# WanqingXia/UR-gym

Measured on AMD Instinct MI355X. Metric: env-steps/sec (whole node), higher is better.
Workload: dtype f64; 1 GPU; UR5DynReach-v1 N=65536 per GPU, random actions U(-1,1), auto-reset, seed 0; envs_total=65536, gather_obs=False, rollout_api=False, gjk_start=bullet

## Files before the change

### ur_gym_amd/csrc/urgym_hip.hip

```cpp
#include <hip/hip_runtime.h>
#include <stdint.h>
#include <stdio.h>
#include <string.h>
#include <math.h>
#include <new>
#include <vector>

#include "../../include/urgym.h"
#include "../../data/ur5e_model.h"
#include "urgym_device.h"
#include "urgym_launch_plan.h"
#include "urgym_actor.h"
#include "urgym_critic.h"
#include "urgym_tables_host.h"

using namespace urgym;


namespace {

constexpr int WAVES = 4;
constexpr int THREADS = GROUP * WAVES;
constexpr uint32_t NO_ITEM = 0xFFFFFFFFu;
constexpr int REFILL_MIN = 16;
constexpr int RESIDENT = 3;
constexpr int SC_ROWS = 19;
constexpr int PAIR_TABLE = 0, PAIR_TRACK = 5, PAIR_SELF = 10;
__host__ __device__ constexpr int self_pair_bit(int la, int lb) {
  return PAIR_SELF + (la == 1 ? 0 : (la == 2 ? 4 : 7)) + (lb - (la + 2));
}

enum { MODE_STEP = 0, MODE_RESET = 1, MODE_REFRESH = 2, MODE_PREFETCH = 3 };
enum { Q_TABLE = 0, Q_TRACK = 1, Q_SELF = 2 };

constexpr double M_HULL = 0.001, M_PRIM = 0.001;
constexpr double CYL_R = 0.05, CYL_H = 0.4, M_CYL = M_PRIM;
constexpr double TABLE_CX = 0.5, TABLE_CY = 0.0, TABLE_CZ = -0.58, TABLE_HX = 0.55, TABLE_HY = 0.9, TABLE_HZ = 0.46;
constexpr double M_TABLE = M_PRIM;
constexpr double TRACK_CX = 0.0, TRACK_CY = 0.0, TRACK_CZ = -0.06, TRACK_HX = 0.1, TRACK_HY = 0.55, TRACK_HZ = 0.06;
constexpr double M_TRACK = M_PRIM;
constexpr double TARGET_BOX_H = 0.025, M_TARGET_BOX = M_PRIM, TARGET_SPHERE_R = 0.02;

struct DevTables {
  double joint_rot[6][9];
  double joint_xyz[6][3];
  double capsule[6][7];
};
__constant__ DevTables c_tab;

constexpr int REC_FIELDS = 36;
enum { REC_GOAL = 0, REC_START = 6, REC_END = 12, REC_VEL = 18, REC_QUAT = 24, REC_LD = 28, REC_DP = 33 };

struct KParams {
  urgym_config cfg;
  urgym_buffers buf;
  HullMap graph;
  int obs_dim, goal_dim;
  uint32_t seed_lo, seed_hi;
  int pp;
  int copy_final;
  int envs;
  int big_blocks;
  int envs_tail;
  double* rec_d;
  int32_t* rec_i;
  int2* rlist;
  int* rcount;
  int rcap;
  double* ld_scratch;
  double* sc_scratch;
  int* rzero;
  int* rzero2;
  int fallback_on;
  int prefetch;
  int inline_ori;
  float neutral_ach[6];
};
__device__ __forceinline__ double& REC(const KParams& P, int slot, int f, int n) {
  return P.rec_d[((size_t)slot * REC_FIELDS + f) * P.cfg.num_envs + n];
}
__device__ __forceinline__ int32_t& RECI(const KParams& P, int slot, int j, int n) {
  return P.rec_i[((size_t)slot * 2 + j) * P.cfg.num_envs + n];
}

__device__ __forceinline__ double& SOA(double* base, int f, int n, int N) { return base[(size_t)f * N + n]; }

__device__ __forceinline__ long long sortable(double x) {
  const long long k = __double_as_longlong(x);
  return k ^ ((k >> 63) & 0x7FFFFFFFFFFFFFFFLL);
}
__device__ __forceinline__ double unsortable(long long k) { return __longlong_as_double(k ^ ((k >> 63) & 0x7FFFFFFFFFFFFFFFLL)); }

__device__ __forceinline__ ShapeDesc hull_desc(int link ) {
  ShapeDesc s;
  s.type = SH_HULL; s.hull = link - 1; s.hx = s.hy = s.hz = 0.0;
  return s;
}
__device__ __forceinline__ ShapeDesc cyl_desc() {
  ShapeDesc s;
  s.type = SH_CYLZ; s.hull = 0;
  s.hx = s.hy = CYL_R - M_CYL; s.hz = 0.5 * CYL_H - M_CYL;
  return s;
}
__device__ __forceinline__ ShapeDesc box_desc(double hx, double hy, double hz, double margin) {
  ShapeDesc s;
  s.type = SH_BOX; s.hull = 0;
  s.hx = hx - margin; s.hy = hy - margin; s.hz = hz - margin;
  return s;
}
// ... 282 lines not shown
    integrate_obstacle(opos, oq, ovel, dp, cfg.dt);
  }
  if (KIND == URGYM_ENV_STA) {
    double st[6], en[6];
    bool moving = false;
    for (int i = 0; i < 6; i++) { st[i] = SOA(B.obst_start, i, n, N); en[i] = SOA(B.obst_end, i, n, N); moving = moving || en[i] != 0.0; }
    if (moving) {
      const double dx = en[0] - opos[0], dy = en[1] - opos[1], dz = en[2] - opos[2];
      double ovel[6] = {0, 0, 0, 0, 0, 0}, dp[3];
      if (sqrt(dx * dx + dy * dy + dz * dz) > 0.05) dyn_velocity(st, en, 1.0, ovel);
      step_displacement(ovel, cfg.dt, dp);
      integrate_obstacle(opos, oq, ovel, dp, cfg.dt);
    }
  }
}

template <int MODE>
struct EnvLds {
  static constexpr int ME = (MODE == MODE_PREFETCH) ? PREFETCH_MAX_ENVS : ((MODE == MODE_STEP) ? STEP_MAX_ENVS : MAX_ENVS);
  static constexpr bool LDS_Q = (MODE == MODE_REFRESH);
  static constexpr bool DIST_LDS = (MODE != MODE_STEP);
  static constexpr bool LDS_STATE = (MODE != MODE_STEP);
  double s_dist[5][DIST_LDS ? ME : 1];
  double s_q[LDS_Q ? 6 : 1][LDS_Q ? ME : 1];
  double s_obst[LDS_STATE ? 7 : 1][LDS_STATE ? ME : 1];
  uint32_t s_pairs[ME];
  int s_flags[ME];
  int s_env[ME];
  alignas(16) int s_ticket;
  int s_pending;
  int s_p1done;
  int s_left;
  int s_key[(MODE != MODE_STEP) ? ME : 1];
  double s_kind[(MODE == MODE_STEP) ? 8 : 1][5];
  double s_pose[GJK_SLOT_DOUBLES][THREADS];
};

template <int KIND, int MODE, bool WITH_EPA>
__device__ __forceinline__ void env_body(const KParams& P, const float* __restrict__ actions, EnvLds<MODE>& L, const int bidx, const int nblk) {
  constexpr int ME = EnvLds<MODE>::ME;
  constexpr bool LDS_Q = EnvLds<MODE>::LDS_Q, DIST_LDS = EnvLds<MODE>::DIST_LDS, LDS_STATE = EnvLds<MODE>::LDS_STATE;
  auto& s_dist = L.s_dist;
  auto& s_q = L.s_q;
  auto& s_obst = L.s_obst;
  auto& s_pairs = L.s_pairs;
  auto& s_flags = L.s_flags;
  auto& s_env = L.s_env;
  int& s_ticket = L.s_ticket;
  int& s_pending = L.s_pending;
  int& s_p1done = L.s_p1done;
  int& s_left = L.s_left;
  auto& s_key = L.s_key;
  auto& s_pose = L.s_pose;

  const urgym_config& cfg = P.cfg;
  const urgym_buffers& B = P.buf;
  const int N = cfg.num_envs;
  const int tid = threadIdx.x;
  const int lane = tid & 63;
  const int wv = __builtin_amdgcn_readfirstlane(tid >> 6);
  constexpr int OD = (KIND == URGYM_ENV_ORI) ? 18 : ((KIND == URGYM_ENV_OBS) ? 26 : ((KIND == URGYM_ENV_STA) ? 29 : 35));
  constexpr int GD = (KIND == URGYM_ENV_OBS) ? 3 : 6;
  int vb = bidx;
  if (MODE == MODE_STEP && P.envs_tail == 0) {
    const int nb = nblk, x = vb & 7, per = nb >> 3, rem = nb & 7;
    vb = x * per + (x < rem ? x : rem) + (vb >> 3);
  }
  const bool tail_block = (MODE == MODE_STEP) && P.envs_tail > 0 && vb >= P.big_blocks;
  const int E = tail_block ? P.envs_tail : P.envs;
  const int first = tail_block ? P.big_blocks * P.envs + (vb - P.big_blocks) * P.envs_tail : vb * P.envs;
  const int G = (E + GROUP - 1) / GROUP;
  constexpr bool HAS_OBST = (KIND != URGYM_ENV_ORI);
  constexpr int COLL_BIT = 1 << 30;
  constexpr int EE_BIT = 1 << 29;
  constexpr int EPA_SHIFT = 8, EPA_MASK = 0x7FFF << EPA_SHIFT;
  const bool need_epa = WITH_EPA && ((KIND == URGYM_ENV_OBS) || !cfg.check_collision || (MODE != MODE_STEP));
  XRef pose_slot{(URGYM_LDS double*)&s_pose[0][0] + tid, THREADS};
  float* const s_out = reinterpret_cast<float*>(&s_pose[0][0]);
  static_assert(sizeof(float) * STEP_MAX_ENVS * 47 <= sizeof(double) * GJK_SLOT_DOUBLES * THREADS, "staging must fit");
  auto dist_cell = [&](int i, int e) -> double* {
    return DIST_LDS ? (double*)&s_dist[i][DIST_LDS ? e : 0] : &P.ld_scratch[(size_t)i * N + first + e];
  };

  if (bidx == 0 && tid == 0) {
    if (P.rzero) *P.rzero = 0;
    if (P.rzero2) *P.rzero2 = 0;
  }
  int list_count = 0;
  if (MODE != MODE_STEP) {
    list_count = (MODE == MODE_PREFETCH) ? min(*P.rcount, P.rcap) : B.done_count[P.pp];
    if (first >= list_count) return;
  }
  if (tid == 0) { s_ticket = THREADS; s_pending = 0; s_p1done = 0; s_left = 0; }
  if (MODE == MODE_STEP && tid < 8) {
    const int k = tid & 3, ex = tid >> 2;
    const bool tbl = (k == Q_TABLE);
    const double msum = M_HULL + ((k == 3) ? M_CYL : ((k == Q_SELF) ? M_HULL : (tbl ? M_TABLE : M_TRACK)));
    const bool wants = (k == 3) || ex;
    const double verdict = wants ? 0.0 : msum + cfg.collision_margin;
    L.s_kind[tid][0] = (k == 3) ? (CYL_R - M_CYL) : (tbl ? (TABLE_HX - M_TABLE) : (TRACK_HX - M_TRACK));
    L.s_kind[tid][1] = (k == 3) ? (CYL_R - M_CYL) : (tbl ? (TABLE_HY - M_TABLE) : (TRACK_HY - M_TRACK));
    L.s_kind[tid][2] = (k == 3) ? (0.5 * CYL_H - M_CYL) : (tbl ? (TABLE_HZ - M_TABLE) : (TRACK_HZ - M_TRACK));
    L.s_kind[tid][3] = wants ? msum + 0.02 + 5.0 : verdict;
    L.s_kind[tid][4] = verdict;
  }
  const bool workbench = (KIND != URGYM_ENV_ORI) && cfg.link_dist_scope == URGYM_LINK_DIST_WORKBENCH;
  if (workbench && tid < E && (DIST_LDS || first + tid < N))
    for (int i = 0; i < 5; i++) *dist_cell(i, tid) = __longlong_as_double(0x7FF0000000000000LL);
  if (MODE == MODE_STEP && tid < E) {
    s_env[tid] = (first + tid < N) ? first + tid : -1;
    s_flags[tid] = 0;
    s_pairs[tid] = 0;
  }
  __syncthreads();
  const int p1_slot = (MODE == MODE_STEP) ? (wv - (WAVES - G)) * GROUP + lane : lane;
  const bool p1_lane = ((MODE == MODE_STEP) ? (wv >= WAVES - G) : (wv == 0)) && (p1_slot < E);
  int n_slot = -1, flags_slot = 0;
  int key_slot = 0;
  if (p1_lane) {
    const int idx = first + p1_slot;
    if (MODE == MODE_STEP) n_slot = idx < N ? idx : -1;
    else if (MODE == MODE_PREFETCH) {
      if (idx < list_count) { const int2 ent = P.rlist[idx]; n_slot = ent.x; key_slot = ent.y; }
    } else n_slot = idx < list_count ? B.done_list[idx] : -1;
  }
  if ((MODE == MODE_RESET || MODE == MODE_PREFETCH) && wv == 0) {
    int episode_used = 0;
    sample_episode_wave<KIND>(P, pose_slot, E, lane, n_slot, key_slot, MODE == MODE_PREFETCH, flags_slot, episode_used);
    if (p1_lane) s_key[p1_slot] = (MODE == MODE_PREFETCH) ? key_slot : episode_used + 1;
  }
  if (p1_lane) {
    const int e = p1_slot;
    const int n = n_slot;
    int flags = flags_slot;
    double q[6] = {0, 0, 0, 0, 0, 0};
    double opos[3] = {0, 0, 0};
    Q4 oq{0, 0, 0, 1};
    bool finite = true;
    if (n >= 0) {
      for (int i = 0; i < 6; i++) q[i] = joint_of_step<MODE>(P, actions, n, i);
      for (int i = 0; i < 6; i++) finite = finite && (fabs(q[i]) < 1.0e6);
      if (MODE == MODE_STEP) {
        bool over = false;
        for (int i = 0; i < 6; i++) over = over || (fabs(q[i]) > (i == 2 ? 3.141592653589793 : 6.283185307179586));
        if (over) atomicOr(&s_flags[p1_slot], URGYM_STATUS_JOINT_LIMIT);
      }
      if (HAS_OBST && LDS_STATE) {
        double sp[6];
        for (int i = 0; i < 6; i++) sp[i] = (MODE == MODE_PREFETCH) ? REC(P, key_slot & 1, REC_START + i, n) : SOA(B.obst_start, i, n, N);
        for (int i = 0; i < 3; i++) opos[i] = sp[i];
        oq = quat_from_rpy(sp[3], sp[4], sp[5]);
      }
    }
    const bool live = (n >= 0 && finite);
    const bool use_cache = (MODE == MODE_STEP) && (HAS_OBST || cfg.check_collision);
    if (use_cache && live) {
#pragma unroll 1
      for (int k = 0; k < 6; k++) {
        double sn, cs;
        sincos(joint_of_step<MODE>(P, actions, n, k), &sn, &cs);
        SOA(P.sc_scratch, 2 * k, n, N) = sn;
        SOA(P.sc_scratch, 2 * k + 1, n, N) = cs;
      }
      if (HAS_OBST) {
        obstacle_of_step<KIND>(P, n, opos, oq);
        for (int i = 0; i < 3; i++) SOA(P.sc_scratch, 12 + i, n, N) = opos[i];
        SOA(P.sc_scratch, 15, n, N) = oq.x; SOA(P.sc_scratch, 16, n, N) = oq.y; SOA(P.sc_scratch, 17, n, N) = oq.z; SOA(P.sc_scratch, 18, n, N) = oq.w;
      }
    }
    s_env[e] = live ? n : (n >= 0 ? -2 - n : -1);
    if (MODE != MODE_STEP) s_flags[e] = flags;
    if (LDS_STATE) {
      if (LDS_Q) for (int i = 0; i < 6; i++) s_q[i][e] = q[i];
      s_obst[0][e] = opos[0]; s_obst[1][e] = opos[1]; s_obst[2][e] = opos[2];
      s_obst[3][e] = oq.x; s_obst[4][e] = oq.y; s_obst[5][e] = oq.z; s_obst[6][e] = oq.w;
    }
    if (HAS_OBST && !live && (DIST_LDS || n >= 0))
      for (int i = 0; i < 5; i++) *dist_cell(i, e) = (n >= 0) ? __builtin_nan("") : 1e30;
    uint32_t pairs = 0;
    if (live && cfg.check_collision && MODE != MODE_RESET && MODE != MODE_PREFETCH) {
      const double lim = cfg.collision_margin + M_HULL + 1e-6;
      X3 T = identity_x3();
      D3 a0[3], a1[3];
#pragma unroll
      for (int k = 0; k < 6; k++) {
        double sn, cs;
        if (use_cache) { sn = SOA(P.sc_scratch, 2 * k, n, N); cs = SOA(P.sc_scratch, 2 * k + 1, n, N); }
        else sincos(q[k], &sn, &cs);
        fk_joint(T, k, sn, cs);
        const int link = k + 1;
        const double* c = c_tab.capsule[k];
        const D3 b0 = apply(T, d3(c[0], c[1], c[2])), b1 = apply(T, d3(c[3], c[4], c[5]));
        const double rb = c[6];
        if (k < 3) { a0[k] = b0; a1[k] = b1; }
        if (link >= 2) {
          if (seg_box_lower_bound(b0, b1, TABLE_CX, TABLE_CY, TABLE_CZ, TABLE_HX, TABLE_HY, TABLE_HZ) - rb <= lim) pairs |= 1u << (PAIR_TABLE + link - 2);
          if (seg_box_lower_bound(b0, b1, TRACK_CX, TRACK_CY, TRACK_CZ, TRACK_HX, TRACK_HY, TRACK_HZ) - rb <= lim) pairs |= 1u << (PAIR_TRACK + link - 2);
        }
#pragma unroll
        for (int A = 1; A <= 3; A++) {
          if (A <= link - 2) {
            if (segseg_dist(a0[A - 1], a1[A - 1], b0, b1) - c_tab.capsule[A - 1][6] - rb <= lim + M_HULL) pairs |= 1u << self_pair_bit(A, link);
          }
        }
      }
      if (MODE == MODE_STEP) {
        double er, ep, ey;
        rpy_from_quat(rot_to_quat(T.r), er, ep, ey);
        float* orow = B.observation + (size_t)n * OD;
        orow[0] = (float)T.t.x; orow[1] = (float)T.t.y; orow[2] = (float)T.t.z;
        orow[3] = (float)er; orow[4] = (float)ep; orow[5] = (float)ey;
        atomicOr(&s_flags[e], EE_BIT);
      }
    }
    s_pairs[e] = pairs;
    if (pairs) atomicAdd(&s_pending, __popc(pairs));
  }
  if (MODE == MODE_STEP) {
    if (wv >= WAVES - G && lane == 0) __hip_atomic_fetch_add(&s_p1done, 1, __ATOMIC_RELEASE, __HIP_MEMORY_SCOPE_WORKGROUP);
  } else {
    __syncthreads();
  }

  if (!(MODE == MODE_STEP && !HAS_OBST && !cfg.check_collision)) {
    D3 v0 = d3(0, 1, 0);
    int kind = 3, e = 0, lb = 2, la = 1;
    auto shape_a = [&]() -> ShapeDesc { return hull_desc(kind == Q_SELF ? la : lb); };
    auto shape_b = [&]() -> ShapeDesc {
      ShapeDesc s;
      s.type = (kind == 3) ? SH_CYLZ : ((kind == Q_SELF) ? SH_HULL : SH_BOX);
      s.hull = lb - 1;
      const bool tbl = (kind == Q_TABLE);
      s.hx = (kind == 3) ? (CYL_R - M_CYL) : (tbl ? (TABLE_HX - M_TABLE) : (TRACK_HX - M_TRACK));
      s.hy = (kind == 3) ? (CYL_R - M_CYL) : (tbl ? (TABLE_HY - M_TABLE) : (TRACK_HY - M_TRACK));
      s.hz = (kind == 3) ? (0.5 * CYL_H - M_CYL) : (tbl ? (TABLE_HZ - M_TABLE) : (TRACK_HZ - M_TRACK));
      return s;
    };
    bool exact = false;
    const bool guided = cfg.gjk_start == URGYM_GJK_START_GUIDED;
    auto capsule_mid = [&](int link, const X3& TX) -> D3 {
      const double* c = c_tab.capsule[link - 1];
      return apply(TX, d3(0.5 * (c[0] + c[3]), 0.5 * (c[1] + c[4]), 0.5 * (c[2] + c[5])));
    };
    auto guided_axis = [&](D3 mid, D3 centre) -> D3 {
      const D3 d = mid - centre;
      const double n2 = dot(d, d);
      return n2 > 1e-12 ? d * (1.0 / sqrt(n2)) : d3(0, 1, 0);
    };
    bool p1_ok = false;
    auto setup = [&](uint32_t item) -> bool {
      e = item & 255;
      kind = (item >> 8) & 3;
      exact = ((item >> 16) & 1) != 0;
      lb = (item >> 10) & 7;
      la = (item >> 13) & 7;
      if (e >= E || lb < 1 || lb > 6 || (kind == Q_SELF && (la < 1 || la > 6))) return false;
      const int n = s_env[e];
      if (n < 0) return false;
      const bool cached = (MODE == MODE_STEP) && p1_ok;
      if (MODE == MODE_STEP && !cached) {
        bool finite = true;
        for (int k = 0; k < 6; k++) finite = finite && (fabs(joint_of_step<MODE>(P, actions, n, k)) < 1.0e6);
        if (!finite) return false;
      }
      X3 T = identity_x3(), TA = identity_x3();
#pragma unroll 1
      for (int k = 0; k < lb; k++) {
        double sn, cs;
        if (cached) { sn = SOA(P.sc_scratch, 2 * k, n, N); cs = SOA(P.sc_scratch, 2 * k + 1, n, N); }
        else sincos(LDS_Q ? s_q[k][e] : joint_of_step<MODE>(P, actions, n, k), &sn, &cs);
        fk_joint(T, k, sn, cs);
        if (k + 1 == la) TA = T;
      }
      if (kind == 3) {
        X3 To;
        if (LDS_STATE) {
          quat_to_rot(Q4{s_obst[3][e], s_obst[4][e], s_obst[5][e], s_obst[6][e]}, To.r);
          To.t = d3(s_obst[0][e], s_obst[1][e], s_obst[2][e]);
        } else if (cached) {
          quat_to_rot(Q4{SOA(P.sc_scratch, 15, n, N), SOA(P.sc_scratch, 16, n, N), SOA(P.sc_scratch, 17, n, N), SOA(P.sc_scratch, 18, n, N)}, To.r);
          To.t = d3(SOA(P.sc_scratch, 12, n, N), SOA(P.sc_scratch, 13, n, N), SOA(P.sc_scratch, 14, n, N));
        } else {
          double op[3];
          Q4 oqs;
          obstacle_of_step<KIND>(P, n, op, oqs);
          quat_to_rot(oqs, To.r);
          To.t = d3(op[0], op[1], op[2]);
        }
        store(pose_slot, rel(To, T));
        v0 = rotT(To, guided ? guided_axis(capsule_mid(lb, T), To.t) : d3(0, 1, 0));
      } else if (kind == Q_SELF) {
        store(pose_slot, rel(T, TA));
        v0 = rotT(T, guided ? guided_axis(capsule_mid(la, TA), capsule_mid(lb, T)) : d3(0, 1, 0));
      } else {
        const bool tbl = (kind == Q_TABLE);
        const D3 centre = d3(tbl ? TABLE_CX : TRACK_CX, tbl ? TABLE_CY : TRACK_CY, tbl ? TABLE_CZ : TRACK_CZ);
        v0 = guided ? guided_axis(capsule_mid(lb, T), centre) : d3(0, 1, 0);
        T.t = T.t - centre;
        store(pose_slot, T);
      }
      return true;
    };
    auto claim_pair = [&]() -> uint32_t {
      int pe = tid % E;
#pragma unroll 1
      for (int trip = 0; trip < 2 * ME; trip++, pe = (pe + 1 == E ? 0 : pe + 1)) {
        uint32_t m = s_pairs[pe];
        while (m) {
          const int b = __ffs((int)m) - 1;
          const uint32_t old = atomicAnd(&s_pairs[pe], ~(1u << b));
          if (old & (1u << b)) {
            if (b < PAIR_TRACK) return (uint32_t)pe | (Q_TABLE << 8) | ((uint32_t)(b - PAIR_TABLE + 2) << 10);
            if (b < PAIR_SELF) return (uint32_t)pe | (Q_TRACK << 8) | ((uint32_t)(b - PAIR_TRACK + 2) << 10);
            const int i = b - PAIR_SELF;
            const int la = i < 4 ? 1 : (i < 7 ? 2 : 3);
            const int l2 = i < 4 ? 3 + i : (i < 7 ? i : i - 2);
            return (uint32_t)pe | (Q_SELF << 8) | ((uint32_t)l2 << 10) | ((uint32_t)la << 13);
          }
          m = old & ~(1u << b);
        }
      }
      return NO_ITEM;
    };
    auto margin_sum = [&]() -> double {
      return M_HULL + ((kind == 3) ? M_CYL : ((kind == Q_SELF) ? M_HULL : ((kind == Q_TABLE) ? M_TABLE : M_TRACK)));
    };
    const int n_tickets = HAS_OBST ? (workbench ? 15 : 5) * E : 0;
    auto ticket_item = [&](int t) -> uint32_t {
      const int body = t / (5 * E), r = t - body * 5 * E;
      const int tl = r / E, te = r - tl * E, link = 2 + tl;
      if (body == 0) return (uint32_t)te | (3u << 8) | ((uint32_t)link << 10);
      return (uint32_t)te | ((uint32_t)(body == 1 ? Q_TABLE : Q_TRACK) << 8) | ((uint32_t)link << 10) | (1u << 16);
    };

    GjkRun run;
    bool busy = false;
    if (MODE == MODE_STEP) p1_ok = __hip_atomic_load(&s_p1done, __ATOMIC_ACQUIRE, __HIP_MEMORY_SCOPE_WORKGROUP) >= G;
    if (tid < n_tickets) {
      busy = setup(ticket_item(tid));
      if (busy) gjk_begin(run, v0);
    }
    for (;;) {
      if (busy) {
        if (MODE == MODE_STEP) {
          const URGYM_LDS double* row = (const URGYM_LDS double*)(URGYM_LDS void*)&L.s_kind[kind | ((int)exact << 2)][0];
          ShapeDesc sb;
          sb.type = (kind == 3) ? SH_CYLZ : ((kind == Q_SELF) ? SH_HULL : SH_BOX);
          sb.hull = lb - 1;
          sb.hx = row[0]; sb.hy = row[1]; sb.hz = row[2];
          gjk_iterate(run, P.graph, shape_a(), pose_slot, sb, row[3], row[4]);
        } else {
          const bool wants_distance = (kind == 3 || exact);
          const double verdict_d = wants_distance ? 0.0 : margin_sum() + cfg.collision_margin;
          gjk_iterate(run, P.graph, shape_a(), pose_slot, shape_b(), wants_distance ? margin_sum() + 0.02 + 5.0 : verdict_d, verdict_d);
        }
        if (run.done) {
          const double msum = margin_sum();
          if (kind == 3 || exact) {
            double dist = run.core - msum;
            if (run.info & GJK_PENETRATING) {
              dist = -msum;
              const int body = (kind == 3) ? 0 : (kind == Q_TABLE ? 1 : 2);
              atomicOr(&s_flags[e], URGYM_STATUS_PENETRATION | (need_epa ? (1 << (EPA_SHIFT + 5 * body + (lb - 2))) : 0));
            }
            if (run.info & GJK_ITERCAP) atomicOr(&s_flags[e], URGYM_STATUS_GJK_ITER);
            if (workbench) atomicMin(reinterpret_cast<long long*>(dist_cell(lb - 2, e)), sortable(dist));
            else *dist_cell(lb - 2, e) = dist;
          } else {
            const bool hit = (run.info & (GJK_PENETRATING | GJK_CLOSE)) || (!(run.info & GJK_SEPARATED) && (run.core - msum) <= cfg.collision_margin);
            if (hit) atomicOr(&s_flags[e], COLL_BIT);
          }
          busy = false;
        }
      }
      typedef int pool_words __attribute__((ext_vector_type(4)));
      const pool_words pool = *(volatile URGYM_LDS pool_words*)(URGYM_LDS void*)&s_ticket;
      __builtin_amdgcn_fence(__ATOMIC_ACQUIRE, "workgroup");
      const bool more_tickets = pool.x < n_tickets;
      const bool p1_published = (MODE != MODE_STEP) || pool.z >= G;
      const bool more_pairs = pool.y > 0;
      if (MODE == MODE_STEP) p1_ok = p1_published;
      const int idle_lanes = __popcll(__ballot(!busy));
      if (!busy && (idle_lanes >= REFILL_MIN || idle_lanes == 64)) {
        uint32_t item = NO_ITEM;
        if (more_tickets) {
          const int t = atomicAdd(&s_ticket, 1);
          if (t < n_tickets) item = ticket_item(t);
        } else if (more_pairs) {
          if (atomicSub(&s_pending, 1) > 0) item = claim_pair();
        }
        if (item != NO_ITEM) {
          busy = setup(item);
          if (busy) gjk_begin(run, v0);
        }
      }
      if (__ballot(busy) == 0ull && !more_tickets && !more_pairs && p1_published) break;
    }
    auto epa_pass = [&]() -> bool {
      const EpaWs ws{(URGYM_LDS double*)&s_pose[0][0] + GROUP * wv, THREADS};
      bool armed = false;
#pragma unroll 1
      for (int g = 0; g < G; g++) {
        const int sl = g * GROUP + lane;
        const int marks = (sl < E) ? ((__hip_atomic_load(&s_flags[sl], __ATOMIC_RELAXED, __HIP_MEMORY_SCOPE_WORKGROUP) & EPA_MASK) >> EPA_SHIFT) : 0;
        unsigned long long envs_marked = __ballot(marks != 0);
#pragma unroll 1
        while (envs_marked) {
          const int el = __builtin_ctzll(envs_marked);
          envs_marked &= envs_marked - 1ull;
          const int ee = g * GROUP + el;
          int me = __shfl(marks, el);
#pragma unroll 1
          while (me) {
            const int b = __builtin_ctz((unsigned)me);
            me &= me - 1;
            int mine = 0;
            if (lane == 0) mine = (atomicAnd(&s_flags[ee], ~(1 << (EPA_SHIFT + b))) >> (EPA_SHIFT + b)) & 1;
            if (!__shfl(mine, 0)) continue;
            if (!armed) {
              pose_slot.p = ws.base;
              if (MODE == MODE_STEP) p1_ok = true;
              armed = true;
            }
            const int body = b / 5, link = 2 + b - 5 * body;
            const uint32_t item = (uint32_t)ee | ((uint32_t)(body == 0 ? 3 : (body == 1 ? Q_TABLE : Q_TRACK)) << 8) | ((uint32_t)link << 10) |
                                  ((body ? 1u : 0u) << 16);
            if (!setup(item)) continue;
            epa_wave_sync();
            bool capped;
            const double depth = epa_wave(P.graph, shape_a(), shape_b(), ws, lane, capped);
            if (lane == 0) {
              const double dist = -(depth + margin_sum());
              if (workbench) atomicMin(reinterpret_cast<long long*>(dist_cell(lb - 2, e)), sortable(dist));
              else *dist_cell(lb - 2, e) = dist;
              if (capped) atomicOr(&s_flags[e], URGYM_STATUS_GJK_ITER);
            }
          }
        }
      }
      if (armed) pose_slot.p = (URGYM_LDS double*)&s_pose[0][0] + tid;
      return armed;
    };
    if (HAS_OBST && WITH_EPA) {
      if (lane == 0) __hip_atomic_fetch_add(&s_left, 1, __ATOMIC_RELEASE, __HIP_MEMORY_SCOPE_WORKGROUP);
#pragma unroll 1
      for (;;) {
        const int left = __hip_atomic_load(&s_left, __ATOMIC_ACQUIRE, __HIP_MEMORY_SCOPE_WORKGROUP);
        const bool served = epa_pass();
        if (!served && left >= WAVES) break;
        if (!served) __builtin_amdgcn_s_sleep(16);
      }
    }
    __syncthreads();
  }

  const int pe = (wv - (WAVES - G)) * GROUP + lane;
  if (wv >= WAVES - G && pe < E && s_env[pe] != -1) {
    const int n = s_env[pe] >= 0 ? s_env[pe] : -2 - s_env[pe];
    double q[6];
    for (int i = 0; i < 6; i++) q[i] = LDS_Q ? s_q[i][pe] : joint_of_step<MODE>(P, actions, n, i);
    const bool ee_ready = (MODE == MODE_STEP) && (s_flags[pe] & EE_BIT);
    X3 TE = identity_x3();
    if (!ee_ready) {
      if (KIND == URGYM_ENV_ORI) {
        double sn[6], cs[6];
#pragma unroll
        for (int k = 0; k < 6; k++) sincos(q[k], &sn[k], &cs[k]);
#pragma unroll
        for (int k = 0; k < 6; k++) fk_joint(TE, k, sn[k], cs[k]);
      } else {
#pragma unroll 1
        for (int k = 0; k < 6; k++) {
          double sn, cs;
          sincos(q[k], &sn, &cs);
          fk_joint(TE, k, sn, cs);
        }
      }
    }
    double opos[3] = {0, 0, 0};
    Q4 oq{0, 0, 0, 1};
    if (HAS_OBST) {
      if (LDS_STATE) {
        opos[0] = s_obst[0][pe]; opos[1] = s_obst[1][pe]; opos[2] = s_obst[2][pe];
        oq = Q4{s_obst[3][pe], s_obst[4][pe], s_obst[5][pe], s_obst[6][pe]};
      } else if (s_env[pe] >= 0) {
        for (int i = 0; i < 3; i++) opos[i] = SOA(P.sc_scratch, 12 + i, n, N);
        oq = Q4{SOA(P.sc_scratch, 15, n, N), SOA(P.sc_scratch, 16, n, N), SOA(P.sc_scratch, 17, n, N), SOA(P.sc_scratch, 18, n, N)};
      } else {
        obstacle_of_step<KIND>(P, n, opos, oq);
      }
    }
    const int step_count = B.step_count[n];
    float* row = &s_out[pe * 47];
    float ach[6];
    if (ee_ready) {
      for (int i = 0; i < 6; i++) ach[i] = B.observation[(size_t)n * OD + i];
    } else {
      Q4 eq = rot_to_quat(TE.r);
      double er, ep, ey;
      rpy_from_quat(eq, er, ep, ey);
      ach[0] = (float)TE.t.x; ach[1] = (float)TE.t.y; ach[2] = (float)TE.t.z;
      ach[3] = (float)er; ach[4] = (float)ep; ach[5] = (float)ey;
    }
    double goal[6];
    for (int i = 0; i < 6; i++) goal[i] = SOA(B.goal, i, n, N);
    double ld_old[5] = {0, 0, 0, 0, 0}, ld_new[5] = {0, 0, 0, 0, 0};
    bool coll = (s_flags[pe] & COLL_BIT) != 0;
    if (HAS_OBST) {
      for (int i = 0; i < 5; i++) {
        ld_new[i] = workbench ? unsortable(__double_as_longlong(*dist_cell(i, pe))) : *dist_cell(i, pe);
        if (MODE == MODE_STEP) ld_old[i] = SOA(B.link_dist, i, n, N);
        if (cfg.check_collision && ld_new[i] <= cfg.collision_margin) coll = true;
      }
    }
    if (MODE == MODE_PREFETCH) {
      const int key = s_key[pe], sl = key & 1;
      int rflags = s_flags[pe] & ~(COLL_BIT | EE_BIT | EPA_MASK);
      if (coll) rflags |= URGYM_STATUS_RESET_COLLISION;
      if (HAS_OBST) {
        for (int i = 0; i < 5; i++) REC(P, sl, REC_LD + i, n) = ld_new[i];
        REC(P, sl, REC_QUAT + 0, n) = oq.x; REC(P, sl, REC_QUAT + 1, n) = oq.y; REC(P, sl, REC_QUAT + 2, n) = oq.z; REC(P, sl, REC_QUAT + 3, n) = oq.w;
        double vel[6] = {0, 0, 0, 0, 0, 0};
        if (KIND == URGYM_ENV_DYN) {
          double st[6], en[6];
          for (int i = 0; i < 6; i++) { st[i] = REC(P, sl, REC_START + i, n); en[i] = REC(P, sl, REC_END + i, n); }
          dyn_velocity(st, en, cfg.dyn_time_duration, vel);
        }
        double dp[3];
        step_displacement(vel, cfg.dt, dp);
        for (int i = 0; i < 6; i++) REC(P, sl, REC_VEL + i, n) = vel[i];
        for (int i = 0; i < 3; i++) REC(P, sl, REC_DP + i, n) = dp[i];
      }
      RECI(P, sl, 1, n) = rflags;
      __threadfence();
      RECI(P, sl, 0, n) = key;
    }
// ... 623 lines not shown

int do_masked(Handle* h, const uint8_t* mask, int mode, hipStream_t s) {
  const int N = h->cfg.num_envs;
  HIP_TRY(h, hipMemsetAsync(h->buf.done_count + h->pp, 0, sizeof(int32_t), s));
  hipLaunchKernelGGL(build_list_kernel, dim3((N + 255) / 256), dim3(256), 0, s, mask, N, h->buf.done_list, h->buf.done_count + h->pp);
  KParams P = make_params(h, 0);
  if (mode == MODE_RESET) {
    const bool pf = h->plan.fused;
    if (pf) {
      if (!h->rec_seed_valid || h->rec_seed != h->seed) {
        HIP_TRY(h, hipMemsetAsync(h->d_reci, 0xFF, sizeof(int32_t) * 4 * (size_t)N, s));
        h->rec_seed = h->seed;
        h->rec_seed_valid = true;
        h->dirty_steps = h->cfg.max_episode_steps + 1;
      } else if (mask != nullptr) {
        KParams Pp = P;
        use_list(h, Pp, (h->parity + 2) % 3);
        launch_mode<MODE_PREFETCH>(h, Pp, nullptr, s, PREFETCH_MAX_ENVS, h->plan.rl_cap[0]);
      }
      HIP_TRY(h, hipMemsetAsync(h->d_rcount, 0, 5 * sizeof(int), s));
      use_list(h, P, 3);
    }
    launch_mode<MODE_RESET>(h, P, nullptr, s, GROUP);
    if (pf) {
      launch_mode<MODE_PREFETCH>(h, P, nullptr, s, 8, h->plan.rl_cap[3]);
      if (mask == nullptr) h->dirty_steps = 0;
    }
    if (mask == nullptr) h->steps_since_full_reset = 0;
  } else {
    launch_mode<MODE_REFRESH>(h, P, nullptr, s, GROUP);
  }
  HIP_TRY(h, hipMemsetAsync(h->buf.done_count, 0, 2 * sizeof(int32_t), s));
  HIP_TRY(h, hipGetLastError());
  h->observed = true;
  return URGYM_OK;
}


int plan_handle(Handle* h, const Tuning& t) {
  h->k = kernels_for(h->cfg);
  h->plan = plan_paths(h->cfg.env_kind, h->cfg.num_envs, h->cfg.auto_reset != 0, t);
  int cus = 256, per_cu = RESIDENT;
  hipDeviceGetAttribute(&cus, hipDeviceAttributeMultiprocessorCount, h->device);
  const hipError_t oe = h->plan.fused ? hipOccupancyMaxActiveBlocksPerMultiprocessor(&per_cu, h->k.fused, THREADS, 0)
                                      : hipOccupancyMaxActiveBlocksPerMultiprocessor(&per_cu, h->k.mode[MODE_STEP], THREADS, 0);
  if (oe != hipSuccess || per_cu < 1) per_cu = RESIDENT;
  if (per_cu > RESIDENT) per_cu = RESIDENT;
  plan_grids(h->plan, cus, per_cu, t);
  const LaunchPlan& p = h->plan;
  if (t.verbose) {
    fprintf(stderr, "[urgym] device %d: %d CUs x %d resident step workgroups; N = %d -> %d envs per step workgroup (%d of them, then %d envs each), %d per reset workgroup\n[urgym] prefetched episode records: %s\n",
            h->device, cus, per_cu, p.num_envs, p.step_envs, p.big_blocks > 0 ? p.big_blocks : p.step_blocks, p.tail_envs, p.reset_envs, p.prefetch ? "on" : "off");
  }
  if (!step_geometry_ok(p)) return fail(h, URGYM_ERR_STATE, "urgym_create: the step launch geometry does not cover the envs exactly once");
  return URGYM_OK;
}

int upload_tables(Handle* h) {
  const HostTables* tabs = nullptr;
  try {
    tabs = &build_host_tables();
  } catch (const std::exception& ex) {
    char msg[256];
    snprintf(msg, sizeof(msg), "urgym_create: building the support map failed: %s", ex.what());
    return fail(h, URGYM_ERR_STATE, msg);
  }
  if (!tabs->ok) return fail(h, URGYM_ERR_STATE, "urgym_create: support map has more records than a 16-bit cell code addresses");
  DevTables t;
  memcpy(t.joint_rot, UR5E_JOINT_ROT, sizeof(t.joint_rot));
  memcpy(t.joint_xyz, UR5E_JOINT_XYZ, sizeof(t.joint_xyz));
  memcpy(t.capsule, UR5E_CAPSULE, sizeof(t.capsule));
  HIP_TRY(h, hipMemcpyToSymbol(HIP_SYMBOL(c_tab), &t, sizeof(t)));
  const size_t rec_bytes = tabs->recs.size() * sizeof(CandRec), cell_bytes = tabs->cell.size() * sizeof(unsigned short);
  HIP_TRY(h, hipMalloc((void**)&h->d_recs, rec_bytes));
  HIP_TRY(h, hipMemcpy(h->d_recs, tabs->recs.data(), rec_bytes, hipMemcpyHostToDevice));
  HIP_TRY(h, hipMalloc((void**)&h->d_cell, cell_bytes));
  HIP_TRY(h, hipMemcpy(h->d_cell, tabs->cell.data(), cell_bytes, hipMemcpyHostToDevice));
  return URGYM_OK;
}

int allocate_scratch(Handle* h) {
  const size_t n = (size_t)h->cfg.num_envs;
  HIP_TRY(h, hipMalloc((void**)&h->d_ld_scratch, sizeof(double) * 5 * n));
  HIP_TRY(h, hipMalloc((void**)&h->d_sc_scratch, sizeof(double) * SC_ROWS * n));
  if (!h->plan.prefetch) return URGYM_OK;
  HIP_TRY(h, hipMalloc((void**)&h->d_rec, sizeof(double) * 2 * REC_FIELDS * n));
  HIP_TRY(h, hipMalloc((void**)&h->d_reci, sizeof(int32_t) * 4 * n));
  for (int i = 0; i < 4; i++) HIP_TRY(h, hipMalloc((void**)&h->d_rl[i], sizeof(int2) * (size_t)h->plan.rl_cap[i]));
  HIP_TRY(h, hipMalloc((void**)&h->d_rcount, sizeof(int) * 5));
  return forget_records(h);
}

int eval_neutral_pose(Handle* h) {
  double* dq = nullptr;
  hipError_t e = hipMalloc((void**)&dq, sizeof(double) * 9);
  if (e == hipSuccess) e = hipMemcpy(dq, h->cfg.neutral_q, sizeof(double) * 6, hipMemcpyHostToDevice);
  if (e == hipSuccess) {
    hipLaunchKernelGGL(ee_pose_kernel, dim3(1), dim3(1), 0, 0, dq, (float*)(dq + 6));
    e = hipMemcpy(h->neutral_ach, dq + 6, sizeof(float) * 6, hipMemcpyDeviceToHost);
  }
  if (dq) hipFree(dq);
  return e == hipSuccess ? URGYM_OK : fail(h, URGYM_ERR_HIP, "urgym_create: neutral pose", e);
}



Actor* find_actor(Handle* h, void* actor) {
  for (Actor* a : h->actors)
    if (a == actor) return a;
  return nullptr;
}

int actor_features(const Handle* h) { return h->obs_dim + 2 * h->goal_dim; }

ActorEnv actor_env(const Handle* h) {
  const urgym_buffers& b = h->buf;
  return ActorEnv{h->cfg.num_envs, h->obs_dim, h->goal_dim, h->cfg.auto_reset, b.observation, b.achieved_goal, b.desired_goal,
                  b.reward, b.final_observation, b.terminated, b.truncated, b.is_success, b.collision};
}

ActorPass actor_pass(const Handle* h, Actor* a, const urgym_trajectory& t, int k, int num_steps) {
  const size_t n = (size_t)h->cfg.num_envs, od = (size_t)h->obs_dim, gd = (size_t)h->goal_dim;
  const size_t pre = (size_t)k * n, post = (size_t)(k > 0 ? k - 1 : 0) * n;
  auto at = [](auto* p, size_t off) { return p ? p + off : p; };
  ActorPass r;
  r.obs = at(t.observation, pre * od), r.ach = at(t.achieved_goal, pre * gd), r.des = at(t.desired_goal, pre * gd);
  r.reward = at(t.reward, post);
  r.terminated = at(t.terminated, post), r.truncated = at(t.truncated, post), r.is_success = at(t.is_success, post);
  r.collision = at(t.collision, post);
  r.final_obs = at(t.final_observation, post * od);
  r.ep_return = t.episode_return, r.ep_last = t.episode_last_step, r.ep_success = t.episode_success;
  const bool summary = t.episode_return || t.episode_last_step || t.episode_success || t.episode_done;
  r.ep_done = t.episode_done ? t.episode_done : (summary ? actor_done_scratch(a) : nullptr);
  r.k = k, r.num_steps = num_steps;
  return r;
}

int enter_actor(Handle* h, void* actor, const char* who, Actor** out) {
  if (int rc = enter_bound(h)) return rc;
  char msg[200];
  Actor* a = find_actor(h, actor);
  if (!a) {
    snprintf(msg, sizeof(msg), "%s: not an actor of this handle (actors belong to the handle they were created with)", who);
    return fail(h, URGYM_ERR_ARG, msg);
  }
  if (actor_in_features(a) != actor_features(h)) {
    snprintf(msg, sizeof(msg), "%s: the actor takes %d features, this env kind offers %d", who, actor_in_features(a), actor_features(h));
    return fail(h, URGYM_ERR_ARG, msg);
  }
  if (!h->observed) {
    snprintf(msg, sizeof(msg), "%s: no observations yet: call urgym_reset (or urgym_refresh) first", who);
    return fail(h, URGYM_ERR_STATE, msg);
  }
  *out = a;
  return URGYM_OK;
}

int check_sampling(Handle* h, const Actor* a, const urgym_sampling* how, bool wants_density, const char* who) {
  char msg[200];
  const char* what = nullptr;
  if (!how) what = "null sampling description";
  else if (how->reserved0 != 0) what = "urgym_sampling.reserved0 must be 0";
  else if (how->mode != URGYM_SAMPLE_MEAN && how->mode != URGYM_SAMPLE_GAUSSIAN && how->mode != URGYM_SAMPLE_UNIFORM)
    what = "unknown sampling mode (URGYM_SAMPLE_MEAN, _GAUSSIAN or _UNIFORM)";
  else if (!actor_has_log_std(a) && (how->mode == URGYM_SAMPLE_GAUSSIAN || (how->mode == URGYM_SAMPLE_MEAN && wants_density)))
    what = "the actor has no log_std head (urgym_actor_set_log_std)";
  if (!what) return URGYM_OK;
// ... 427 lines not shown
```

Baseline: 320.8 million env-steps/s.

## Precompute obstacle-relative link poses in phase one for pooled GJK setup

```diff
diff --git a/ur_gym_amd/csrc/urgym_hip.hip b/ur_gym_amd/csrc/urgym_hip.hip
--- a/ur_gym_amd/csrc/urgym_hip.hip
+++ b/ur_gym_amd/csrc/urgym_hip.hip
@@ -4,6 +4,7 @@
 #include <string.h>
 #include <math.h>
 #include <new>
+#include <type_traits>
 #include <vector>
 
 #include "../../include/urgym.h"
@@ -22,9 +23,14 @@
 constexpr int WAVES = 4;
 constexpr int THREADS = GROUP * WAVES;
 constexpr uint32_t NO_ITEM = 0xFFFFFFFFu;
-constexpr int REFILL_MIN = 16;
+#ifndef URGYM_REFILL_MIN
+#define URGYM_REFILL_MIN 16
+#endif
+constexpr int REFILL_MIN = URGYM_REFILL_MIN;
+static_assert(REFILL_MIN >= 1 && REFILL_MIN <= 64, "a wave has 64 lanes");
 constexpr int RESIDENT = 3;
 constexpr int SC_ROWS = 19;
+constexpr int SC_OP_ROWS = 15, SC_ROWS_ALL = SC_ROWS + 5 * SC_OP_ROWS;
 constexpr int PAIR_TABLE = 0, PAIR_TRACK = 5, PAIR_SELF = 10;
 __host__ __device__ constexpr int self_pair_bit(int la, int lb) {
   return PAIR_SELF + (la == 1 ? 0 : (la == 2 ? 4 : 7)) + (lb - (la + 2));
@@ -473,6 +479,16 @@
     return DIST_LDS ? (double*)&s_dist[i][DIST_LDS ? e : 0] : &P.ld_scratch[(size_t)i * N + first + e];
   };
 
+  const bool guided = cfg.gjk_start == URGYM_GJK_START_GUIDED;
+  auto capsule_mid = [&](int link, const X3& TX) -> D3 {
+    const double* c = c_tab.capsule[link - 1];
+    return apply(TX, d3(0.5 * (c[0] + c[3]), 0.5 * (c[1] + c[4]), 0.5 * (c[2] + c[5])));
+  };
+  auto guided_axis = [&](D3 mid, D3 centre) -> D3 {
+    const D3 d = mid - centre;
+    const double n2 = dot(d, d);
+    return n2 > 1e-12 ? d * (1.0 / sqrt(n2)) : d3(0, 1, 0);
+  };
   if (bidx == 0 && tid == 0) {
     if (P.rzero) *P.rzero = 0;
     if (P.rzero2) *P.rzero2 = 0;
@@ -559,6 +575,30 @@
         SOA(P.sc_scratch, 15, n, N) = oq.x; SOA(P.sc_scratch, 16, n, N) = oq.y; SOA(P.sc_scratch, 17, n, N) = oq.z; SOA(P.sc_scratch, 18, n, N) = oq.w;
       }
     }
+    const bool file_ops = (MODE == MODE_STEP) && HAS_OBST && use_cache && live && (4 * E + e >= THREADS);
+    X3 To = identity_x3();
+    if (file_ops) {
+      quat_to_rot(oq, To.r);
+      To.t = d3(opos[0], opos[1], opos[2]);
+    }
+    auto file_operands = [&](int tl, const X3& T) {
+      if (tl * E + e < THREADS) return;
+      double* const row = &SOA(P.sc_scratch, SC_ROWS + SC_OP_ROWS * tl, n, N);
+      const X3 C = rel(To, T);
+      const D3 v = rotT(To, guided ? guided_axis(capsule_mid(2 + tl, T), To.t) : d3(0, 1, 0));
+#pragma unroll
+      for (int k = 0; k < 9; k++) row[(size_t)k * N] = C.r[k];
+      row[(size_t)9 * N] = C.t.x; row[(size_t)10 * N] = C.t.y; row[(size_t)11 * N] = C.t.z;
+      row[(size_t)12 * N] = v.x; row[(size_t)13 * N] = v.y; row[(size_t)14 * N] = v.z;
+    };
+    if (file_ops && !cfg.check_collision) {
+      X3 T = identity_x3();
+#pragma unroll 1
+      for (int k = 0; k < 6; k++) {
+        fk_joint(T, k, SOA(P.sc_scratch, 2 * k, n, N), SOA(P.sc_scratch, 2 * k + 1, n, N));
+        if (k >= 1) file_operands(k - 1, T);
+      }
+    }
     s_env[e] = live ? n : (n >= 0 ? -2 - n : -1);
     if (MODE != MODE_STEP) s_flags[e] = flags;
     if (LDS_STATE) {
@@ -579,6 +619,7 @@
         if (use_cache) { sn = SOA(P.sc_scratch, 2 * k, n, N); cs = SOA(P.sc_scratch, 2 * k + 1, n, N); }
         else sincos(q[k], &sn, &cs);
         fk_joint(T, k, sn, cs);
+        if (k >= 1 && file_ops) file_operands(k - 1, T);
         const int link = k + 1;
         const double* c = c_tab.capsule[k];
         const D3 b0 = apply(T, d3(c[0], c[1], c[2])), b1 = apply(T, d3(c[3], c[4], c[5]));
@@ -628,18 +669,8 @@
       return s;
     };
     bool exact = false;
-    const bool guided = cfg.gjk_start == URGYM_GJK_START_GUIDED;
-    auto capsule_mid = [&](int link, const X3& TX) -> D3 {
-      const double* c = c_tab.capsule[link - 1];
-      return apply(TX, d3(0.5 * (c[0] + c[3]), 0.5 * (c[1] + c[4]), 0.5 * (c[2] + c[5])));
-    };
-    auto guided_axis = [&](D3 mid, D3 centre) -> D3 {
-      const D3 d = mid - centre;
-      const double n2 = dot(d, d);
-      return n2 > 1e-12 ? d * (1.0 / sqrt(n2)) : d3(0, 1, 0);
-    };
     bool p1_ok = false;
-    auto setup = [&](uint32_t item) -> bool {
+    auto setup = [&](uint32_t item, auto pooled) -> bool {
       e = item & 255;
       kind = (item >> 8) & 3;
       exact = ((item >> 16) & 1) != 0;
@@ -653,6 +684,18 @@
         bool finite = true;
         for (int k = 0; k < 6; k++) finite = finite && (fabs(joint_of_step<MODE>(P, actions, n, k)) < 1.0e6);
         if (!finite) return false;
+      }
+      if (MODE == MODE_STEP && HAS_OBST && decltype(pooled)::value) {
+        if (cached && kind == 3 && (lb - 2) * E + e >= THREADS) {
+          const double* const row = &SOA(P.sc_scratch, SC_ROWS + SC_OP_ROWS * (lb - 2), n, N);
+          double w[SC_OP_ROWS];
+#pragma unroll
+          for (int k = 0; k < SC_OP_ROWS; k++) w[k] = row[(size_t)k * N];
+#pragma unroll
+          for (int k = 0; k < 12; k++) pose_slot.set(k, w[k]);
+          v0 = d3(w[12], w[13], w[14]);
+          return true;
+        }
       }
       X3 T = identity_x3(), TA = identity_x3();
 #pragma unroll 1
@@ -728,7 +771,7 @@
     bool busy = false;
     if (MODE == MODE_STEP) p1_ok = __hip_atomic_load(&s_p1done, __ATOMIC_ACQUIRE, __HIP_MEMORY_SCOPE_WORKGROUP) >= G;
     if (tid < n_tickets) {
-      busy = setup(ticket_item(tid));
+      busy = setup(ticket_item(tid), std::false_type{});
       if (busy) gjk_begin(run, v0);
     }
     for (;;) {
@@ -781,7 +824,7 @@
           if (atomicSub(&s_pending, 1) > 0) item = claim_pair();
         }
         if (item != NO_ITEM) {
-          busy = setup(item);
+          busy = setup(item, std::true_type{});
           if (busy) gjk_begin(run, v0);
         }
       }
@@ -816,7 +859,7 @@
             const int body = b / 5, link = 2 + b - 5 * body;
             const uint32_t item = (uint32_t)ee | ((uint32_t)(body == 0 ? 3 : (body == 1 ? Q_TABLE : Q_TRACK)) << 8) | ((uint32_t)link << 10) |
                                   ((body ? 1u : 0u) << 16);
-            if (!setup(item)) continue;
+            if (!setup(item, std::false_type{})) continue;
             epa_wave_sync();
             bool capped;
             const double depth = epa_wave(P.graph, shape_a(), shape_b(), ws, lane, capped);
@@ -1632,7 +1675,7 @@
 int allocate_scratch(Handle* h) {
   const size_t n = (size_t)h->cfg.num_envs;
   HIP_TRY(h, hipMalloc((void**)&h->d_ld_scratch, sizeof(double) * 5 * n));
-  HIP_TRY(h, hipMalloc((void**)&h->d_sc_scratch, sizeof(double) * SC_ROWS * n));
+  HIP_TRY(h, hipMalloc((void**)&h->d_sc_scratch, sizeof(double) * SC_ROWS_ALL * n));
   if (!h->plan.prefetch) return URGYM_OK;
   HIP_TRY(h, hipMalloc((void**)&h->d_rec, sizeof(double) * 2 * REC_FIELDS * n));
   HIP_TRY(h, hipMalloc((void**)&h->d_reci, sizeof(int32_t) * 4 * n));
```

Result: no change. 322.7 million env-steps/s (median of 6 runs) (+0.6%).

## Split step epilogue to overlap observation staging with collision passes

Applied to the files above, without the earlier changes.

```diff
diff --git a/ur_gym_amd/csrc/urgym_hip.hip b/ur_gym_amd/csrc/urgym_hip.hip
--- a/ur_gym_amd/csrc/urgym_hip.hip
+++ b/ur_gym_amd/csrc/urgym_hip.hip
@@ -613,6 +613,13 @@
     __syncthreads();
   }
 
+  constexpr bool SPLIT = (MODE == MODE_STEP) && !WITH_EPA && (KIND == URGYM_ENV_DYN || KIND == URGYM_ENV_STA);
+  static_assert(sizeof(float) * GROUP * 47 <= sizeof(double) * GJK_SLOT_DOUBLES * GROUP, "a wave's rows must fit its own slot share");
+  auto stage = [&](int f) -> float& { return s_out[((f >> 7) * THREADS + GROUP * wv) * 2 + (f & 127)]; };
+  int e_n = -1, e_step_count = 0;
+  bool e_succ = false;
+  double e_d = 0.0, e_th = 0.0, e_q[6] = {0, 0, 0, 0, 0, 0}, e_opos[3] = {0, 0, 0}, e_ld_old[5] = {0, 0, 0, 0, 0};
+  Q4 e_oq{0, 0, 0, 1};
   if (!(MODE == MODE_STEP && !HAS_OBST && !cfg.check_collision)) {
     D3 v0 = d3(0, 1, 0);
     int kind = 3, e = 0, lb = 2, la = 1;
@@ -842,7 +849,177 @@
         if (!served) __builtin_amdgcn_s_sleep(16);
       }
     }
+    if (SPLIT && wv >= WAVES - G) {
+      const int g = wv - (WAVES - G);
+      const int pe = g * GROUP + lane;
+      if (pe < E && s_env[pe] != -1) {
+        const int n = s_env[pe] >= 0 ? s_env[pe] : -2 - s_env[pe];
+        e_n = n;
+        for (int i = 0; i < 6; i++) e_q[i] = joint_of_step<MODE>(P, actions, n, i);
+        const bool ee_ready = (__hip_atomic_load(&s_flags[pe], __ATOMIC_RELAXED, __HIP_MEMORY_SCOPE_WORKGROUP) & EE_BIT) != 0;
+        if (s_env[pe] >= 0) {
+          for (int i = 0; i < 3; i++) e_opos[i] = SOA(P.sc_scratch, 12 + i, n, N);
+          e_oq = Q4{SOA(P.sc_scratch, 15, n, N), SOA(P.sc_scratch, 16, n, N), SOA(P.sc_scratch, 17, n, N), SOA(P.sc_scratch, 18, n, N)};
+        } else {
+          obstacle_of_step<KIND>(P, n, e_opos, e_oq);
+        }
+        e_step_count = B.step_count[n];
+        float ach[6];
+        if (ee_ready) {
+          for (int i = 0; i < 6; i++) ach[i] = B.observation[(size_t)n * OD + i];
+        } else {
+          X3 TE = identity_x3();
+#pragma unroll 1
+          for (int k = 0; k < 6; k++) {
+            double sn, cs;
+            sincos(e_q[k], &sn, &cs);
+            fk_joint(TE, k, sn, cs);
+          }
+          Q4 eq = rot_to_quat(TE.r);
+          double er, ep, ey;
+          rpy_from_quat(eq, er, ep, ey);
+          ach[0] = (float)TE.t.x; ach[1] = (float)TE.t.y; ach[2] = (float)TE.t.z;
+          ach[3] = (float)er; ach[4] = (float)ep; ach[5] = (float)ey;
+        }
+        double goal[6];
+        for (int i = 0; i < 6; i++) goal[i] = SOA(B.goal, i, n, N);
+        for (int i = 0; i < 5; i++) e_ld_old[i] = SOA(B.link_dist, i, n, N);
+        double vobs[6] = {0, 0, 0, 0, 0, 0};
+        if (KIND == URGYM_ENV_DYN && e_step_count < cfg.dyn_motion_steps)
+          for (int i = 0; i < 6; i++) vobs[i] = SOA(B.obst_vel, i, n, N);
+        const int f0 = lane * 47;
+        int p = 0;
+        for (int i = 0; i < 6; i++) stage(f0 + p++) = ach[i];
+        for (int i = 0; i < 6; i++) stage(f0 + p++) = (float)e_q[i];
+        for (int i = 0; i < 6; i++) stage(f0 + p++) = (float)goal[i];
+        for (int i = 0; i < 3; i++) stage(f0 + p++) = (float)e_opos[i];
+        double r_, p_, y_;
+        rpy_from_quat(e_oq, r_, p_, y_);
+        stage(f0 + p++) = (float)r_; stage(f0 + p++) = (float)p_; stage(f0 + p++) = (float)y_;
+        if (KIND == URGYM_ENV_DYN)
+          for (int i = 0; i < 6; i++) stage(f0 + p++) = (float)vobs[i];
+        for (int i = 0; i < 5; i++) stage(f0 + p++) = (float)e_ld_old[i];
+        for (int i = 0; i < GD; i++) { stage(f0 + OD + i) = ach[i]; stage(f0 + OD + GD + i) = (float)goal[i]; }
+        const double a6[6] = {(double)ach[0], (double)ach[1], (double)ach[2], (double)ach[3], (double)ach[4], (double)ach[5]};
+        e_d = pos_distance(a6, goal);
+        e_th = angular_distance(a6 + 3, goal + 3);
+        e_succ = (e_d < cfg.distance_threshold) && (e_th < cfg.ori_threshold);
+      }
+      epa_wave_sync();
+      const int base = first + g * GROUP;
+      const int cnt = max(0, min(min(E, N - first) - g * GROUP, GROUP));
+      for (int i = lane; i < cnt * OD; i += GROUP) __builtin_nontemporal_store(stage((i / OD) * 47 + (i % OD)), &B.observation[(size_t)base * OD + i]);
+      for (int i = lane; i < cnt * GD; i += GROUP) {
+        __builtin_nontemporal_store(stage((i / GD) * 47 + OD + (i % GD)), &B.achieved_goal[(size_t)base * GD + i]);
+        __builtin_nontemporal_store(stage((i / GD) * 47 + OD + GD + (i % GD)), &B.desired_goal[(size_t)base * GD + i]);
+      }
+    }
     __syncthreads();
+  }
+
+  if (SPLIT) {
+    if (e_n >= 0) {
+      const int n = e_n;
+      const int pe = (wv - (WAVES - G)) * GROUP + lane;
+      const int sflags = s_flags[pe];
+      double ld_new[5];
+      for (int i = 0; i < 5; i++) ld_new[i] = *dist_cell(i, pe);
+      bool coll = (sflags & COLL_BIT) != 0;
+      for (int i = 0; i < 5; i++) {
+        if (workbench) ld_new[i] = unsortable(__double_as_longlong(ld_new[i]));
+        if (cfg.check_collision && ld_new[i] <= cfg.collision_margin) coll = true;
+      }
+      int flags = sflags & ~(COLL_BIT | EE_BIT | EPA_MASK);
+      const bool succ = e_succ;
+      bool terminated = succ || coll;
+      bool info_success = terminated ? !coll : false;
+      double reward = 0.0;
+      bool update_ld = false;
+      if (coll) reward = cfg.w_collision;
+      else if (succ) reward = cfg.w_success;
+      else {
+        reward += cfg.w_distance * e_d;
+        reward += cfg.w_orientation * e_th;
+        double sum = 0.0;
+        for (int i = 0; i < 5; i++) sum += (ld_new[i] < cfg.near_threshold) ? cfg.w_link[i] * (ld_new[i] - e_ld_old[i]) : 0.0;
+        reward += sum;
+        update_ld = true;
+      }
+      if (reward != reward) flags |= URGYM_STATUS_NAN;
+      if (!update_ld) flags &= ~(URGYM_STATUS_PENETRATION | URGYM_STATUS_GJK_ITER);
+      const int sc = e_step_count + 1;
+      bool truncated = sc >= cfg.max_episode_steps;
+      for (int i = 0; i < 6; i++) SOA(B.q, i, n, N) = e_q[i];
+      B.step_count[n] = sc;
+      for (int i = 0; i < 3; i++) SOA(B.obst_pos, i, n, N) = e_opos[i];
+      SOA(B.obst_quat, 0, n, N) = e_oq.x; SOA(B.obst_quat, 1, n, N) = e_oq.y; SOA(B.obst_quat, 2, n, N) = e_oq.z; SOA(B.obst_quat, 3, n, N) = e_oq.w;
+      if (update_ld)
+        for (int i = 0; i < 5; i++) SOA(B.link_dist, i, n, N) = ld_new[i];
+      B.reward[n] = (float)reward;
+      B.terminated[n] = terminated ? 1 : 0;
+      B.truncated[n] = truncated ? 1 : 0;
+      B.is_success[n] = info_success ? 1 : 0;
+      B.collision[n] = coll ? 1 : 0;
+      if (cfg.auto_reset && (terminated || truncated)) {
+        bool consumed = false;
+        if (P.prefetch) {
+          const int ecur = B.episode_id[n], sl = ecur & 1;
+          if (RECI(P, sl, 0, n) == ecur) {
+            consumed = true;
+            const int f0 = lane * 47;
+            for (int i = 0; i < OD; i++) B.final_observation[(size_t)n * OD + i] = stage(f0 + i);
+            for (int i = 0; i < GD; i++) {
+              B.final_achieved_goal[(size_t)n * GD + i] = stage(f0 + OD + i);
+              B.final_desired_goal[(size_t)n * GD + i] = stage(f0 + OD + GD + i);
+            }
+            double g2[6], st2[6], ld2[5], q2[6];
+            for (int i = 0; i < 6; i++) { g2[i] = REC(P, sl, REC_GOAL + i, n); st2[i] = REC(P, sl, REC_START + i, n); q2[i] = cfg.neutral_q[i]; }
+            for (int i = 0; i < 6; i++) { SOA(B.goal, i, n, N) = g2[i]; SOA(B.q, i, n, N) = q2[i]; }
+            for (int i = 0; i < 6; i++) {
+              SOA(B.obst_start, i, n, N) = st2[i];
+              SOA(B.obst_end, i, n, N) = REC(P, sl, REC_END + i, n);
+              SOA(B.obst_vel, i, n, N) = REC(P, sl, REC_VEL + i, n);
+            }
+            for (int i = 0; i < 3; i++) SOA(B.obst_vel, 6 + i, n, N) = REC(P, sl, REC_DP + i, n);
+            const Q4 oq2{REC(P, sl, REC_QUAT + 0, n), REC(P, sl, REC_QUAT + 1, n), REC(P, sl, REC_QUAT + 2, n), REC(P, sl, REC_QUAT + 3, n)};
+            for (int i = 0; i < 3; i++) SOA(B.obst_pos, i, n, N) = st2[i];
+            SOA(B.obst_quat, 0, n, N) = oq2.x; SOA(B.obst_quat, 1, n, N) = oq2.y; SOA(B.obst_quat, 2, n, N) = oq2.z; SOA(B.obst_quat, 3, n, N) = oq2.w;
+            for (int i = 0; i < 5; i++) { ld2[i] = REC(P, sl, REC_LD + i, n); SOA(B.link_dist, i, n, N) = ld2[i]; }
+            B.step_count[n] = 0;
+            B.episode_id[n] = ecur + 1;
+            flags |= RECI(P, sl, 1, n);
+            __builtin_amdgcn_s_waitcnt(0x0F70);
+            __builtin_amdgcn_fence(__ATOMIC_RELEASE, "workgroup");
+            float* obs = B.observation + (size_t)n * OD;
+            int p = 0;
+            for (int i = 0; i < 6; i++) obs[p++] = P.neutral_ach[i];
+            for (int i = 0; i < 6; i++) obs[p++] = (float)q2[i];
+            for (int i = 0; i < 6; i++) obs[p++] = (float)g2[i];
+            for (int i = 0; i < 3; i++) obs[p++] = (float)st2[i];
+            double r_, p_, y_;
+            rpy_from_quat(oq2, r_, p_, y_);
+            obs[p++] = (float)r_; obs[p++] = (float)p_; obs[p++] = (float)y_;
+            if (KIND == URGYM_ENV_DYN)
+              for (int i = 0; i < 6; i++) obs[p++] = (float)(double)stage(f0 + 24 + i);
+            for (int i = 0; i < 5; i++) obs[p++] = (float)ld2[i];
+            for (int i = 0; i < GD; i++) {
+              B.achieved_goal[(size_t)n * GD + i] = P.neutral_ach[i];
+              B.desired_goal[(size_t)n * GD + i] = (float)g2[i];
+            }
+            const int pos = atomicAdd(P.rcount, 1);
+            if (pos < P.rcap) P.rlist[pos] = make_int2(n, ecur + 2);
+          }
+        }
+        if (!consumed) {
+          int slot = atomicAdd(&B.done_count[P.pp], 1);
+          B.done_list[slot] = n;
+          if (P.prefetch && !P.fallback_on) atomicOr(&B.status[n], URGYM_STATUS_STALE_RECORD);
+        }
+      }
+      if (flags) atomicOr(&B.status[n], flags);
+    }
+    if (bidx == 0 && tid == 0) B.done_count[P.pp ^ 1] = 0;
+    return;
   }
 
   const int pe = (wv - (WAVES - G)) * GROUP + lane;
```

After: 320.4 million env-steps/s before, 319.6 million env-steps/s after. Within noise of the previous version (-0.3%).
